# gkaissis/PriMIA

Hardware: AMD Instinct MI355X
Metric: images_per_sec (higher is better)
Workload: dtype bf16; 1 GPU; ResNet-18 federated-client training step (fwd+loss+bwd+SGD), batch 256/client, 3x224x224, 1 client per GPU; batch_per_client=256, clients=1, sync_every_n_batch=3, dp_sgd=False

## Files before the change

include/primia_hip.h:

```cpp
#ifndef PRIMIA_HIP_H
#define PRIMIA_HIP_H

#include <stdint.h>

#ifdef __cplusplus
extern "C" {
#endif

#define PRIMIA_OK 0
#define PRIMIA_ERR_ARG (-1)
#define PRIMIA_ERR_LAUNCH (-2)
#define PRIMIA_ERR_UNSUPPORTED (-3)
#define PRIMIA_ERR_WORKSPACE (-4)
#define PRIMIA_ERR_INTERNAL (-5)

#define PRIMIA_F32 0
#define PRIMIA_BF16 1

typedef void* primia_stream_t;

int primia_abi_version(void);

int primia_set_option(const char* name, int value);
int64_t primia_options_epoch(void);
// ... 21 lines not shown

int64_t primia_conv_wfwd_elems(const primia_conv_desc* d);
int64_t primia_conv_wdgrad_elems(const primia_conv_desc* d);

int primia_conv_weight_prepare(const primia_conv_desc* d, int c_real, const float* w_oihw,
                               void* w_fwd, void* w_dgrad, int dtype, primia_stream_t stream);

int primia_conv_weight_prepare_many(const primia_conv_desc* descs_host, const int* c_real_host,
                                    const float* const* w_oihw_host, void* const* w_fwd_host,
                                    void* const* w_dgrad_host, int n, int dtype, primia_stream_t stream);
int primia_conv_wgrad_finalize_many(const primia_conv_desc* descs_host, const int* c_real_host,
                                    const float* const* dw_acc_host, float* const* dw_oihw_host, int n,
                                    primia_stream_t stream);

int primia_conv_sgd_fusable(const primia_conv_desc* d, int c_real);
int primia_conv_sgd_step_many(const primia_conv_desc* descs_host, const int* c_real_host,
                              const float* const* dw_acc_host, float* const* dw_oihw_host,
                              float* const* w_oihw_host, void* const* w_fwd_host, void* const* w_dgrad_host,
                              int n, float lr, float weight_decay, int dtype, primia_stream_t stream);
int primia_conv_sgd_step_many_dev(const primia_conv_desc* descs_host, const int* c_real_host,
                                  const float* const* dw_acc_host, float* const* dw_oihw_host,
                                  float* const* w_oihw_host, void* const* w_fwd_host, void* const* w_dgrad_host,
                                  int n, const float* hyper, int dtype, primia_stream_t stream);

int primia_conv_fwd_pair_ok(const primia_conv_desc* d, const primia_conv_desc* d_ds, int dtype);
int primia_conv2d_fwd_stats_pair(const primia_conv_desc* d, const void* x, const void* w_fwd, void* y,
                                 float* stat_sums, const primia_conv_desc* d_ds, const void* w_fwd_ds, void* y_ds,
                                 float* stat_sums_ds, int dtype, primia_stream_t stream);

int primia_conv2d_fwd(const primia_conv_desc* d, const void* x, const void* w_fwd, void* y,
                      int dtype, primia_stream_t stream);
int primia_stem_pad_dims(int H, int W, int* Hp, int* Wp);
int primia_stem_conv_fwd(const void* x_padded, const void* w_fwd, void* y, int N, int H, int W, int dtype,
                         primia_stream_t stream);
int primia_stem_conv_stat_slots(int N, int H, int W);
int primia_stem_conv_fwd_stats(const void* x_padded, const void* w_fwd, void* y, float* stat_partials, int N, int H,
                               int W, int dtype, primia_stream_t stream);
int primia_stem_conv_stats(const void* x_padded, const void* w_fwd, float* stat_partials, int N, int H, int W, int dtype,
                           primia_stream_t stream);
int primia_stem_conv_pool_ok(int N, int H, int W, int dtype);
int primia_stem_conv_pool(const void* x_padded, const void* w_fwd, void* y, void* pooled, uint8_t* argmax,
                          const float* gamma, const float* beta, const float* save_mean, const float* save_invstd, int N,
                          int H, int W, int dtype, primia_stream_t stream);
int primia_stem_conv_pool_eval(const void* x_padded, const void* w_fwd, void* pooled, uint8_t* argmax, const float* gamma,
                               const float* beta, const float* running_mean, const float* running_var, float eps, int N,
                               int H, int W, int dtype, primia_stream_t stream);
// ... 288 lines not shown
                              float* ps_dbeta, int N, int HW, int C, void* workspace, int64_t workspace_bytes, int dtype,
                              primia_stream_t stream);

int primia_maxpool3x3s2_fwd(const void* x, void* y, uint8_t* argmax, int N, int H, int W, int C,
                            int dtype, primia_stream_t stream);
int primia_maxpool3x3s2_bwd(const void* dy, const uint8_t* argmax, void* dx, int N, int H, int W,
                            int C, int dtype, primia_stream_t stream);
int primia_avgpool3x3s2_fwd(const void* x, void* y, int N, int H, int W, int C, int dtype,
                            primia_stream_t stream);
int primia_avgpool3x3s2_bwd(const void* dy, void* dx, int N, int H, int W, int C, int dtype,
                            primia_stream_t stream);
int primia_global_avgpool_fwd(const void* x, float* feat, int N, int HW, int C, int dtype,
                              primia_stream_t stream);
int primia_global_avgpool_bwd(const float* dfeat, void* dx, int N, int HW, int C, int dtype,
                              primia_stream_t stream);

int primia_head_fwd(const void* x, const float* w, const float* b, float* feat, float* logits, int N, int HW, int C,
                    int out_f, int dtype, primia_stream_t stream);
int primia_head_bwd(const float* w, const float* dlogits, void* dx, int N, int HW, int C, int out_f, int dtype,
                    primia_stream_t stream);
int primia_head_bwd_bnsums(const float* w, const float* dlogits, void* dx, const void* bn_y, const uint8_t* relu_mask,
                           const float* bn_mean, const float* bn_invstd, float* sums, int N, int HW, int C, int out_f, int dtype,
                           primia_stream_t stream);
int primia_linear_fwd(const float* x, const float* w, const float* b, float* y, int N, int in_f,
                      int out_f, primia_stream_t stream);
int primia_linear_bwd(const float* x, const float* w, const float* dy, float* dx, float* dw,
                      float* db, int N, int in_f, int out_f, primia_stream_t stream);
int primia_xent_hard(const float* logits, const int64_t* target, const float* class_weight,
                     float* loss, float* dlogits, int N, int C, primia_stream_t stream);
int primia_xent_soft(const float* logits, const float* target, const float* class_weight,
                     float* loss, float* dlogits, int N, int C, primia_stream_t stream);

int primia_sgd_step(float* p, const float* g, int64_t n, float lr, float weight_decay,
                    primia_stream_t stream);
int primia_sgd_step_ranges(float* p, const float* g, const int64_t* begin_host, const int64_t* len_host, int n,
                           float lr, float weight_decay, primia_stream_t stream);
int primia_adam_step(float* p, const float* g, float* exp_avg, float* exp_avg_sq, int64_t n,
                     float lr, float beta1, float beta2, float eps, float weight_decay,
                     int64_t step, primia_stream_t stream);

int primia_sgd_step_dev(float* p, const float* g, int64_t n, const float* hyper, primia_stream_t stream);
int primia_sgd_step_ranges_dev(float* p, const float* g, const int64_t* begin_host, const int64_t* len_host, int n,
                               const float* hyper, primia_stream_t stream);
int primia_adam_step_dev(float* p, const float* g, float* exp_avg, float* exp_avg_sq, int64_t n,
                         const float* hyper, primia_stream_t stream);
int primia_opt_hyper_set(float* hyper, float lr, float weight_decay, float beta1, float beta2, float eps,
// ... 139 lines not shown
```

primia_amd/csrc/bn.hip:

```cpp
#include <stdlib.h>

#include "common.h"

namespace primia {

constexpr int kMaxPartialBlocks = 1024;


template <typename T, typename F, int UNROLL = 0>
__global__ __launch_bounds__(256) void colreduce2_kernel(F f, long M, int C, long rows_per_block,
                                                         float* __restrict__ partials) {
    constexpr int CH = Chunk<T>::N;
    const int tpr = C / CH;
    const int rpp = 256 / tpr;
    const int rg = threadIdx.x / tpr, cc = threadIdx.x % tpr;
    const long r0 = (long)blockIdx.x * rows_per_block;
    long r1 = r0 + rows_per_block;
    if (r1 > M) r1 = M;

    float s1[CH], s2[CH];
#pragma unroll
    for (int i = 0; i < CH; ++i) s1[i] = s2[i] = 0.f;
    if (rg < rpp) {
        F lf = f;
// ... 87 lines not shown

constexpr int kFinSlices = 64;
template <int NQ>
__device__ __forceinline__ void fin_gather(const float* __restrict__ partials, int nblk, int C, int c, int ks,
                                           double (&acc)[NQ]) {
    for (int k0 = ks; k0 < nblk; k0 += 8 * kFinSlices) {
        float v[8][NQ];
#pragma unroll
        for (int u = 0; u < 8; ++u) {
            const int k = k0 + u * kFinSlices;
#pragma unroll
            for (int q = 0; q < NQ; ++q) {
                const float t = partials[((long)(k < nblk ? k : nblk - 1) * NQ + q) * C + c];
                v[u][q] = k < nblk ? t : 0.f;
            }
        }
#pragma unroll
        for (int u = 0; u < 8; ++u)
#pragma unroll
            for (int q = 0; q < NQ; ++q) acc[q] += (double)v[u][q];
    }
}

__global__ __launch_bounds__(16 * kFinSlices) void bn_finalize_kernel(const float* __restrict__ partials, int nblk,
                                                          int C, long M, int mode, float eps,
                                                          float momentum, float* out1, float* out2,
                                                          float* running_mean, float* running_var,
                                                          const float* scale2 = nullptr) {
    __shared__ double sa[kFinSlices][17], sb[kFinSlices][17];
    const int cl = threadIdx.x & 15, ks = threadIdx.x >> 4;
    const int c = blockIdx.x * 16 + cl;
    float rm0 = 0.f, rv0 = 0.f, sc2v = 1.f;
    if (ks == 0 && c < C) {
        if (mode == 0 && running_mean) {
            rm0 = running_mean[c];
            rv0 = running_var[c];
        } else if (mode != 0 && scale2) {
            sc2v = scale2[c];
        }
    }
    double acc2[2] = {0.0, 0.0};
    if (c < C) fin_gather<2>(partials, nblk, C, c, ks, acc2);
    double a = acc2[0], b = acc2[1];
    sa[ks][cl] = a;
    sb[ks][cl] = b;
    __syncthreads();
    if (ks >= 4) return;
    for (int k = ks + 4; k < kFinSlices; k += 4) {
        a += sa[k][cl];
        b += sb[k][cl];
    }
    a += __shfl_down(a, 32);
    b += __shfl_down(b, 32);
    a += __shfl_down(a, 16);
    b += __shfl_down(b, 16);
    if (ks != 0 || c >= C) return;
    if (mode == 0) {
        const double mean = a / (double)M;
        double var = b / (double)M - mean * mean;
        if (var < 0.0) var = 0.0;
        out1[c] = (float)mean;
        out2[c] = (float)(1.0 / sqrt(var + (double)eps));
        if (running_mean) {
            const double unb = M > 1 ? var * (double)M / (double)(M - 1) : var;
            running_mean[c] = (float)((1.0 - momentum) * (double)rm0 + (double)momentum * mean);
            running_var[c] = (float)((1.0 - momentum) * (double)rv0 + (double)momentum * unb);
        }
    } else {
        out1[c] = (float)a;
        out2[c] = scale2 ? (float)(b * (double)sc2v) : (float)b;
    }
}

template <typename T>
__global__ __launch_bounds__(16 * kFinSlices) void bn_finalize_pool_kernel(
    const float* __restrict__ partials, int nblk, int C, float* __restrict__ dbeta, float* __restrict__ dgamma,
    const float* __restrict__ gamma, const float* __restrict__ beta, const float* __restrict__ mean,
    const float* __restrict__ invstd, const T* __restrict__ p, const T* __restrict__ dp, const uint8_t* __restrict__ argmax,
    const T* __restrict__ y, int N, int H, int W, int Ho, int Wo) {
    __shared__ double sa[kFinSlices][17], sb[kFinSlices][17];
    __shared__ double sfix[16 * kFinSlices / 64];
    const int cl = threadIdx.x & 15, ks = threadIdx.x >> 4;
    const int c = blockIdx.x * 16 + cl;
    double acc2[2] = {0.0, 0.0};
    if (c < C) fin_gather<2>(partials, nblk, C, c, ks, acc2);
    sa[ks][cl] = acc2[0];
    sb[ks][cl] = acc2[1];
    __syncthreads();
    if (ks == 0 && c < C) {
        double a = 0.0, b = 0.0;
        for (int k = 0; k < kFinSlices; ++k) {
            a += sa[k][cl];
            b += sb[k][cl];
        }
// ... 992 lines not shown
            (const T*)y, (const T*)dpooled, argmax, (T*)dy, gamma, beta, save_mean, save_invstd, dbeta, dgamma,
            (float)(1.0 / (double)M), N, H, W, C, Ho, Wo);
    } else {
        bn_relu_pool_bwd_apply_kernel<T><<<stream_blocks(nchunks) * 2, 256, 0, st>>>(
            (const T*)y, (const T*)dpooled, argmax, (T*)dy, gamma, beta, save_mean, save_invstd, dbeta, dgamma,
            (float)(1.0 / (double)M), N, H, W, C, Ho, Wo, 1.0f / (float)W, 1.0f / (float)H);
    }
    return launch_status();
}

}

using namespace primia;

template <typename T>
static int bn_fwd_train_pair_impl(const void* y2, const void* yd, void* z, uint8_t* relu_mask, const float* gamma2,
                                  const float* beta2, float* rm2, float* rv2, float* sm2, float* si2, const float* sums2,
                                  int slots2, const float* gammad, const float* betad, float* rmd, float* rvd, float* smd,
                                  float* sid, const float* sumsd, int slotsd, long M, int C, float eps, float momentum,
                                  float* ws, hipStream_t st) {
    int nblk;
    long rpb;
    reduce_geometry(M, C, nblk, rpb);
    const float* partd = sumsd;
    int nd = slotsd;
    if (!sumsd) {
        StatsFn<T> fd{(const T*)yd};
        colreduce2_kernel<T, StatsFn<T>><<<nblk, 256, 0, st>>>(fd, M, C, rpb, ws);
        partd = ws;
        nd = nblk;
    }
    bn_finalize_kernel<<<(C + 15) / 16, 16 * kFinSlices, 0, st>>>(partd, nd, C, M, 0, eps, momentum, smd, sid, rmd, rvd);
    const float* part = sums2;
    int n2 = slots2;
    if (!sums2) {
        StatsFn<T> f2{(const T*)y2};
        colreduce2_kernel<T, StatsFn<T>><<<nblk, 256, 0, st>>>(f2, M, C, rpb, ws);
        part = ws;
        n2 = nblk;
    }
    bn_finalize_kernel<<<(C + 15) / 16, 16 * kFinSlices, 0, st>>>(part, n2, C, M, 0, eps, momentum, sm2, si2, rm2, rv2);
    const long nchunks = M * C / Chunk<T>::N;
    bn_apply_pair_kernel<T><<<stream_blocks(nchunks), 256, 0, st>>>((const T*)y2, (const T*)yd, (T*)z, gamma2, beta2, sm2,
                                                                    si2, gammad, betad, smd, sid, nchunks, C, relu_mask);
    return launch_status();
}

extern "C" {

int64_t primia_bn_workspace_bytes(int64_t M, int C) {
    (void)M;
    return (int64_t)kMaxPartialBlocks * 2 * C * sizeof(float);
}

int primia_bn_fwd_train(const void* y, const void* residual, void* z, const float* gamma,
                        const float* beta, float* running_mean, float* running_var,
                        float* save_mean, float* save_invstd, int64_t M, int C, float eps,
                        float momentum, int relu, void* workspace, int64_t workspace_bytes,
                        int dtype, primia_stream_t stream) {
    PRIMIA_REQUIRE(y && z && gamma && beta && save_mean && save_invstd && workspace);
    PRIMIA_REQUIRE((running_mean == nullptr) == (running_var == nullptr));
    PRIMIA_REQUIRE(bn_shape_ok(M, C, dtype));
    if (workspace_bytes < primia_bn_workspace_bytes(M, C)) return PRIMIA_ERR_WORKSPACE;
    hipStream_t st = (hipStream_t)stream;
    if (dtype == PRIMIA_F32)
// ... 403 lines not shown
```

primia_amd/csrc/layout.hip:

```cpp
#include "common.h"
#include "conv_common.h"

namespace primia {

template <typename T>
__global__ __launch_bounds__(256) void nchw_to_nhwc_kernel(const float* __restrict__ src,
                                                           T* __restrict__ dst, int C, int HW,
                                                           int c_pad, long total) {
    long i = (long)blockIdx.x * blockDim.x + threadIdx.x;
    if (i >= total) return;
    long n = i / HW;
    long hw = i - n * HW;
    const float* s = src + n * (long)C * HW + hw;
    T* d = dst + i * c_pad;
    for (int c = 0; c < c_pad; ++c) Elem<T>::store(d + c, c < C ? s[(long)c * HW] : 0.f);
}

template <typename T>
__global__ __launch_bounds__(256) void nchw_to_nhwc_padded_kernel(const float* __restrict__ src, T* __restrict__ dst,
                                                                  int C, int H, int W, int c_pad, int pad_top,
                                                                  int pad_left, int Hp, int Wp, long total) {
    long i = (long)blockIdx.x * blockDim.x + threadIdx.x;
    if (i >= total) return;
    const int HW = H * W;
// ... 360 lines not shown
}

template <typename T>
__global__ __launch_bounds__(256) void conv_sgd_tiled_dev_kernel(SgdTileArgs a, const float* __restrict__ hyper) {
    __shared__ float lds[kTileK9 * (64 * 9 + 1)];
    const float lr = hyper[kHyperLr], wd = hyper[kHyperWd];
    int c = 0;
    while (c + 1 < a.n && (int)blockIdx.x >= a.tile_begin[c + 1]) ++c;
    const SgdTileEntry& en = a.e[c];
    const int tile = blockIdx.x - a.tile_begin[c];
    if (en.RS == 9)
        sgd_tile<T, 9, kTileK9, true>(en, tile, lds, lr, wd);
    else
        sgd_tile<T, 1, 32, true>(en, tile, lds, lr, wd);
}

constexpr int kMaxRanges = 32;
struct SgdRanges {
    long begin[kMaxRanges], len[kMaxRanges];
    int n;
    long total;
};
__device__ __forceinline__ void sgd_ranges_body(float* __restrict__ p, const float* __restrict__ g, const SgdRanges& r,
                                                float lr, float wd) {
    const long stride = (long)gridDim.x * 256;
    for (long i = (long)blockIdx.x * 256 + threadIdx.x; i < r.total; i += stride) {
        long j = i;
        int k = 0;
        while (k + 1 < r.n && j >= r.len[k]) j -= r.len[k++];
        const long o = r.begin[k] + j;
        p[o] = sgd_update(p[o], g[o], lr, wd);
    }
}
__global__ __launch_bounds__(256) void sgd_ranges_kernel(float* __restrict__ p, const float* __restrict__ g, SgdRanges r,
                                                         float lr, float wd) {
    sgd_ranges_body(p, g, r, lr, wd);
}
__global__ __launch_bounds__(256) void sgd_ranges_dev_kernel(float* __restrict__ p, const float* __restrict__ g,
                                                             SgdRanges r, const float* __restrict__ hyper) {
    const float lr = hyper[kHyperLr], wd = hyper[kHyperWd];
    sgd_ranges_body(p, g, r, lr, wd);
}

static inline bool tiled_ok(const ConvGeom& g, int c_real) {
    return !g.stem && c_real == g.C && g.C % 64 == 0 && g.K % 32 == 0 && (g.R * g.S == 9 || g.R * g.S == 1);
}

}

using namespace primia;

extern "C" {

int primia_abi_version(void) { return 1; }

int primia_nchw_to_nhwc(const float* src, void* dst, int N, int C, int H, int W, int c_pad,
                        int dtype, primia_stream_t stream) {
    PRIMIA_REQUIRE(src && dst && N > 0 && C > 0 && H > 0 && W > 0 && c_pad >= C);
    long total = (long)N * H * W;
    dim3 grid(ceil_div(total, 256)), block(256);
    hipStream_t st = (hipStream_t)stream;
    if (dtype == PRIMIA_F32)
        nchw_to_nhwc_kernel<float><<<grid, block, 0, st>>>(src, (float*)dst, C, H * W, c_pad, total);
    else if (dtype == PRIMIA_BF16)
        nchw_to_nhwc_kernel<bf16><<<grid, block, 0, st>>>(src, (bf16*)dst, C, H * W, c_pad, total);
    else
        return PRIMIA_ERR_ARG;
    return launch_status();
// ... 284 lines not shown
}

int primia_sgd_step_ranges(float* p, const float* g, const int64_t* begin_host, const int64_t* len_host, int n, float lr,
                           float weight_decay, primia_stream_t stream) {
    if (n == 0) return PRIMIA_OK;
    SgdRanges r;
    const int rc = sgd_ranges_args(p, g, begin_host, len_host, n, r);
    if (rc != PRIMIA_OK) return rc;
    sgd_ranges_kernel<<<sgd_ranges_blocks(r), 256, 0, (hipStream_t)stream>>>(p, g, r, lr, weight_decay);
    return launch_status();
}

int primia_sgd_step_ranges_dev(float* p, const float* g, const int64_t* begin_host, const int64_t* len_host, int n,
                               const float* hyper, primia_stream_t stream) {
    if (n == 0) return PRIMIA_OK;
    PRIMIA_REQUIRE(hyper);
    SgdRanges r;
    const int rc = sgd_ranges_args(p, g, begin_host, len_host, n, r);
    if (rc != PRIMIA_OK) return rc;
    sgd_ranges_dev_kernel<<<sgd_ranges_blocks(r), 256, 0, (hipStream_t)stream>>>(p, g, r, hyper);
    return launch_status();
}

}
```

primia_amd/csrc/pool_fc_loss.hip:

```cpp
#include "common.h"

namespace primia {

template <typename T, bool IS_MAX>
__global__ __launch_bounds__(256) void pool3x3s2_fwd_kernel(const T* __restrict__ x, T* __restrict__ y,
                                                            uint8_t* __restrict__ argmax, int N, int H,
                                                            int W, int C, int Ho, int Wo) {
    constexpr int CH = Chunk<T>::N;
    const int cpr = C / CH;
    const long total = (long)N * Ho * Wo * cpr;
    const long q = (long)blockIdx.x * 256 + threadIdx.x;
    if (q >= total) return;
    const int cc = (int)(q % cpr);
    long t = q / cpr;
    const int wo = (int)(t % Wo);
    t /= Wo;
    const int ho = (int)(t % Ho);
    const int n = (int)(t / Ho);
    float best[CH];
    int pos[CH];
#pragma unroll
    for (int i = 0; i < CH; ++i) {
        best[i] = IS_MAX ? -INFINITY : 0.f;
        pos[i] = -1;
// ... 116 lines not shown
__global__ __launch_bounds__(64) void linear_fwd_kernel(const float* __restrict__ x, const float* __restrict__ w,
                                                        const float* __restrict__ b, float* __restrict__ y,
                                                        int in_f, int out_f) {
    const int n = blockIdx.x, lane = threadIdx.x;
    for (int j = 0; j < out_f; ++j) {
        float s = 0.f;
        for (int i = lane; i < in_f; i += 64) s += x[(long)n * in_f + i] * w[(long)j * in_f + i];
        s = wave_sum(s);
        if (lane == 0) y[(long)n * out_f + j] = s + (b ? b[j] : 0.f);
    }
}
__global__ __launch_bounds__(256) void linear_bwd_dx_kernel(const float* __restrict__ w,
                                                            const float* __restrict__ dy,
                                                            float* __restrict__ dx, int N, int in_f,
                                                            int out_f) {
    const long i = (long)blockIdx.x * 256 + threadIdx.x;
    if (i >= (long)N * in_f) return;
    const int f = (int)(i % in_f);
    const long n = i / in_f;
    float s = 0.f;
    for (int j = 0; j < out_f; ++j) s += dy[n * out_f + j] * w[(long)j * in_f + f];
    dx[i] = s;
}
__global__ __launch_bounds__(1024) void linear_bwd_dw_kernel(const float* __restrict__ x,
                                                             const float* __restrict__ dy,
                                                             float* __restrict__ dw, float* __restrict__ db,
                                                             int N, int in_f, int out_f) {
    __shared__ float red[16][64];
    const int j = blockIdx.y, i = blockIdx.x * 64 + (threadIdx.x & 63), ng = threadIdx.x >> 6;
    float s = 0.f;
    if (i <= in_f)
        for (int n = ng; n < N; n += 16) s += dy[(long)n * out_f + j] * (i < in_f ? x[(long)n * in_f + i] : 1.f);
    red[ng][threadIdx.x & 63] = s;
    __syncthreads();
    if (ng == 0 && i <= in_f) {
        for (int g = 1; g < 16; ++g) s += red[g][threadIdx.x & 63];
        if (i < in_f)
            dw[(long)j * in_f + i] = s;
        else if (db)
            db[j] = s;
    }
}

template <typename T>
__global__ __launch_bounds__(256) void head_fwd_kernel(const T* __restrict__ x, const float* __restrict__ w,
                                                       const float* __restrict__ b, float* __restrict__ feat,
                                                       float* __restrict__ y, int HW, int C, int out_f) {
    constexpr int CH = Chunk<T>::N;
    extern __shared__ float sh[];
    const int tpr = C / CH, rpp = 256 / tpr;
    const int rg = threadIdx.x / tpr, cc = threadIdx.x % tpr;
    const int n = blockIdx.x;
    float s[CH];
#pragma unroll
    for (int i = 0; i < CH; ++i) s[i] = 0.f;
// ... 29 lines not shown
template <typename T>
__global__ __launch_bounds__(256) void head_bwd_kernel(const float* __restrict__ w, const float* __restrict__ dy,
                                                       T* __restrict__ dx, int HW, int C, int out_f) {
    constexpr int CH = Chunk<T>::N;
    extern __shared__ float sh[];
    const int n = blockIdx.x;
    for (int c = threadIdx.x; c < C; c += 256) {
        float a = 0.f;
        for (int j = 0; j < out_f; ++j) a += dy[(long)n * out_f + j] * w[(long)j * C + c];
        sh[c] = a / (float)HW;
    }
    __syncthreads();
    const int cpr = C / CH;
    for (int q = threadIdx.x; q < HW * cpr; q += 256) {
        const int c0 = (q % cpr) * CH;
        float v[CH];
#pragma unroll
        for (int i = 0; i < CH; ++i) v[i] = sh[c0 + i];
        *(u32x4*)(dx + (long)n * HW * C + (long)q * CH) = Chunk<T>::pack(v);
    }
}

template <typename T>
__global__ __launch_bounds__(256) void head_bwd_bnsums_kernel(const float* __restrict__ w, const float* __restrict__ dy,
                                                              T* __restrict__ dx, const T* __restrict__ bn_y,
                                                              const uint8_t* __restrict__ relu_mask,
                                                              const float* __restrict__ bn_mean,
                                                              const float* __restrict__ bn_invstd, float* __restrict__ sums,
                                                              int HW, int C, int out_f) {
    constexpr int CH = Chunk<T>::N;
    extern __shared__ float sh[];
    const int n = blockIdx.x;
    for (int c = threadIdx.x; c < C; c += 256) {
        float a = 0.f;
        for (int j = 0; j < out_f; ++j) a += dy[(long)n * out_f + j] * w[(long)j * C + c];
        sh[c] = a / (float)HW;
    }
    __syncthreads();
    const int cpr = C / CH;
    const int c0 = (threadIdx.x % cpr) * CH;
    float v[CH], vr[CH], mu[CH], cnt[CH], sx[CH];
#pragma unroll
    for (int i = 0; i < CH; ++i) {
        v[i] = sh[c0 + i];
        mu[i] = bn_mean[c0 + i];
        cnt[i] = sx[i] = 0.f;
    }
    const u32x4 packed = Chunk<T>::pack(v);
    Chunk<T>::unpack(packed, vr);
    for (int q = threadIdx.x; q < HW * cpr; q += 256) {
        const long off = (long)n * HW * C + (long)q * CH;
        *(u32x4*)(dx + off) = packed;
        float yv[CH];
        Chunk<T>::unpack(*(const u32x4*)(bn_y + off), yv);
        const unsigned m = relu_mask[off / CH];
#pragma unroll
        for (int i = 0; i < CH; ++i) {
            const bool on = (m >> i) & 1u;
            cnt[i] += on ? 1.f : 0.f;
            sx[i] += on ? yv[i] - mu[i] : 0.f;
        }
    }
    float* red = sh + C;
    const int grp = threadIdx.x / cpr;
#pragma unroll
    for (int i = 0; i < CH; ++i) {
        red[(grp * 2 + 0) * C + c0 + i] = vr[i] * cnt[i];
        red[(grp * 2 + 1) * C + c0 + i] = vr[i] * sx[i];
    }
    __syncthreads();
    const int ngrp = 256 / cpr;
    for (int c = threadIdx.x; c < 2 * C; c += 256) {
        const int qq = c / C, cc = c - qq * C;
        float a = 0.f;
        for (int g = 0; g < ngrp; ++g) a += red[(g * 2 + qq) * C + cc];
        if (qq) a *= bn_invstd[cc];
        sums[((long)n * 2 + qq) * C + cc] = a;
    }
}

__device__ __forceinline__ float block_sum_256(float v, float* sh) {
    v = wave_sum(v);
    if ((threadIdx.x & 63) == 0) sh[threadIdx.x >> 6] = v;
    __syncthreads();
    const float r = sh[0] + sh[1] + sh[2] + sh[3];
    __syncthreads();
    return r;
}

constexpr int kMaxClasses = 16;

template <bool SOFT>
__global__ __launch_bounds__(256) void xent_kernel(const float* __restrict__ logits, const void* target,
                                                   const float* __restrict__ cw, float* __restrict__ loss,
                                                   float* __restrict__ dlogits, int N, int C) {
    __shared__ float sh[4];
    float num = 0.f, den = 0.f;
    for (int n = threadIdx.x; n < N; n += 256) {
        const float* o = logits + (long)n * C;
        float mx = o[0];
// ... 168 lines not shown
        head_bwd_kernel<bf16><<<N, 256, lds, st>>>(w, dlogits, (bf16*)dx, HW, C, out_f);
    return launch_status();
}

int primia_head_bwd_bnsums(const float* w, const float* dlogits, void* dx, const void* bn_y, const uint8_t* relu_mask,
                           const float* bn_mean, const float* bn_invstd, float* sums, int N, int HW, int C, int out_f, int dtype,
                           primia_stream_t stream) {
    PRIMIA_REQUIRE(w && dlogits && dx && bn_y && relu_mask && bn_mean && bn_invstd && sums && N > 0 && HW > 0 && C > 0 && out_f > 0);
    PRIMIA_REQUIRE((dtype == PRIMIA_F32 || dtype == PRIMIA_BF16) && head_shape_ok(C, dtype));
    const int cpr = C / (dtype == PRIMIA_F32 ? 4 : 8);
    if (cpr > 256 || 256 % cpr) return PRIMIA_ERR_UNSUPPORTED;
    hipStream_t st = (hipStream_t)stream;
    const size_t lds = (size_t)(1 + 2 * (256 / cpr)) * C * sizeof(float);
    if (lds > 48 * 1024) return PRIMIA_ERR_UNSUPPORTED;
    if (dtype == PRIMIA_F32)
        head_bwd_bnsums_kernel<float><<<N, 256, lds, st>>>(w, dlogits, (float*)dx, (const float*)bn_y, relu_mask, bn_mean,
                                                           bn_invstd, sums, HW, C, out_f);
    else
        head_bwd_bnsums_kernel<bf16><<<N, 256, lds, st>>>(w, dlogits, (bf16*)dx, (const bf16*)bn_y, relu_mask, bn_mean,
                                                          bn_invstd, sums, HW, C, out_f);
    return launch_status();
}

int primia_linear_fwd(const float* x, const float* w, const float* b, float* y, int N, int in_f,
                      int out_f, primia_stream_t stream) {
    PRIMIA_REQUIRE(x && w && y && N > 0 && in_f > 0 && out_f > 0);
    linear_fwd_kernel<<<N, 64, 0, (hipStream_t)stream>>>(x, w, b, y, in_f, out_f);
    return launch_status();
}
int primia_linear_bwd(const float* x, const float* w, const float* dy, float* dx, float* dw,
                      float* db, int N, int in_f, int out_f, primia_stream_t stream) {
    PRIMIA_REQUIRE(x && w && dy && dw && N > 0 && in_f > 0 && out_f > 0);
    hipStream_t st = (hipStream_t)stream;
    if (dx) linear_bwd_dx_kernel<<<ceil_div((long)N * in_f, 256), 256, 0, st>>>(w, dy, dx, N, in_f, out_f);
    linear_bwd_dw_kernel<<<dim3((in_f + 1 + 63) / 64, out_f), 1024, 0, st>>>(x, dy, dw, db, N, in_f, out_f);
    return launch_status();
}

int primia_xent_hard(const float* logits, const int64_t* target, const float* class_weight,
                     float* loss, float* dlogits, int N, int C, primia_stream_t stream) {
    PRIMIA_REQUIRE(logits && target && loss && N > 0 && C > 0);
    xent_kernel<false><<<1, 256, 0, (hipStream_t)stream>>>(logits, target, class_weight, loss, dlogits, N, C);
    return launch_status();
}
int primia_xent_soft(const float* logits, const float* target, const float* class_weight,
                     float* loss, float* dlogits, int N, int C, primia_stream_t stream) {
// ... 7 lines not shown
```

primia_amd/engine.py:

```python
import os
from collections import OrderedDict

import torch

from . import _lib
from ._lib import ConvDesc, call, query
from .resnet_spec import NetSpec, bn_name, buffer_entries, init_state_dict, param_entries, resnet18_spec, state_dict_keys

BN_EPS = 1e-5
BN_MOMENTUM = 0.1


class _Conv:
    def __init__(self, spec, desc, c_real):
        self.spec, self.desc, self.c_real = spec, desc, c_real


class ResNet18Engine:
    def __init__(self, batch_size, num_classes=3, in_channels=3, input_size=224, pooling="max",
                 dtype=torch.bfloat16, device="cuda:0", norm="batch", groups=32, options=None, share=None):
        self._root = self if share is None else share._root
        self._options = dict(options or {})
        for k, v in self._options.items():
            if not hasattr(type(self), k):
# ... 785 lines not shown
            smp, sip = self.save[pb2]
            self._timed("dgrad", c1, lambda: call(
                "primia_conv2d_dgrad_pair_bnsums", c1.desc, dy1, c1.w_dgrad, cd.desc, dyd, cd.w_dgrad, dx_in,
                t[prev.prefix + ".y2"], self.relu_masks[pb2], smp, sip, sums, self.dt), extra_macs=self._macs(cd))
            self._dout_sums[prev.prefix] = (sums, pslots)
        else:
            self._timed("dgrad", c1, lambda: call("primia_conv2d_dgrad_pair", c1.desc, dy1, c1.w_dgrad, cd.desc, dyd,
                                                  cd.w_dgrad, dx_in, self.dt), extra_macs=self._macs(cd))

    def backward(self):
        N, t = self.N, self.t
        nc = self.spec.num_classes
        if query("primia_options_epoch") != self._options_epoch:
            raise _lib.PrimiaError("library options changed (primia_set_option) after this engine sized its buffers")
        self._grads_pending = False
        self._wg_seen = {}
        self._dout_sums = {}
        if self.wgrad_ws is not None and self.dp is None:
            stem_overwrites = self._acc_zero_only_stem and self._stem_bwd_fused_wanted()
            if not stem_overwrites:
                self.dw_acc[:self._acc_zero_n].zero_()
        else:
            self.dw_acc.zero_()
        call("primia_linear_bwd", self.feat, self.views["fc.weight"], self.dlogits, None,
             self._gviews["fc.weight"], self._gviews["fc.bias"], N, 512, nc)
        last = self.spec.blocks[-1].prefix
        hw = self.final_hw
        blocks = self.spec.blocks
        lb2 = bn_name(blocks[-1].conv2.name)
        if (self.norm == "batch" and self.dp is None and blocks[-1].down is None and lb2 in self.relu_masks
                and self._head_bnsums_ok()):
            sums = self._bwd_sums("head", N, 512)
            sml, sil = self.save[lb2]
            call("primia_head_bwd_bnsums", self.views["fc.weight"], self.dlogits, t[last + ".dout"], t[last + ".y2"],
                 self.relu_masks[lb2], sml, sil, sums, N, hw * hw, 512, nc, self.dt)
            self._dout_sums[last] = (sums, N)
        else:
            call("primia_head_bwd", self.views["fc.weight"], self.dlogits, t[last + ".dout"], N, hw * hw, 512, nc, self.dt)
        for i in range(len(blocks) - 1, -1, -1):
            blk, prev = blocks[i], (blocks[i - 1] if i > 0 else None)
            x_in = t[prev.prefix + ".out"] if prev is not None else t["pool.out"]
            dx_in = t[prev.prefix + ".dout"] if prev is not None else t["pool.dout"]
            if self.taps is not None:
                self.taps[blk.prefix + ".dout_in"] = t[blk.prefix + ".dout"].clone()
            if blk.down is None:
                self._backward_identity(blk, prev, x_in, dx_in)
            else:
                self._backward_transition(blk, prev, x_in, dx_in)
        hw = self.stem_hw
        stem_bwd_fused = self._stem_bwd_fused_wanted()
        self.stem_bwd_fused_active = stem_bwd_fused
        pool_sums, self._pool_sums = getattr(self, "_pool_sums", None), None
        if stem_bwd_fused:
            sm, si = self.save["bn1"]
            c = self.convs["conv1"]
            S = self.spec.input_size
            if pool_sums is not None:
                call("primia_bn_relu_maxpool_bwd_from_sums", t["stem.y"], t["pool.out"], t["pool.dout"], self.pool_argmax,
                     self.views["bn1.weight"], self.views["bn1.bias"], sm, si, self._gviews["bn1.weight"],
                     self._gviews["bn1.bias"], pool_sums[0], pool_sums[1], N, hw, hw, 64, self.dt)
# ... 89 lines not shown
    def _sgd_tail_plan(self):
        if getattr(self, "_sgd_plan", None) is None:
            import ctypes

            cs = list(self.convs.values())
            fus = [c for c in cs if query("primia_conv_sgd_fusable", c.desc, c.c_real) == 1 and c.w_dgrad is not None
                   and all(tt.data_ptr() % 16 == 0 for tt in (c.acc, c.w_fwd, c.w_dgrad, self.views[c.spec.name + ".weight"],
                                                              self._gviews[c.spec.name + ".weight"]))]
            rest = [c for c in cs if c not in fus]
            vp = lambda t: ctypes.c_void_p(t.data_ptr()) if t is not None else ctypes.c_void_p(0)

            def pack(lst):
                n = len(lst)
                if n == 0:
                    return None
                return dict(
                    n=n, descs=(ConvDesc * n)(*[c.desc for c in lst]), creal=(ctypes.c_int * n)(*[c.c_real for c in lst]),
                    w=(ctypes.c_void_p * n)(*[vp(self.views[c.spec.name + ".weight"]) for c in lst]),
                    wf=(ctypes.c_void_p * n)(*[vp(c.w_fwd) for c in lst]),
                    wd=(ctypes.c_void_p * n)(*[vp(c.w_dgrad) for c in lst]),
                    acc=(ctypes.c_void_p * n)(*[vp(c.acc) for c in lst]),
                    gw=(ctypes.c_void_p * n)(*[vp(self._gviews[c.spec.name + ".weight"]) for c in lst]))

            fused_keys = {c.spec.name + ".weight" for c in fus}
            ranges, off = [], 0
            for k, shp in self.p_entries:
                n = int(torch.Size(shp).numel())
                if k not in fused_keys:
                    if ranges and ranges[-1][0] + ranges[-1][1] == off:
                        ranges[-1][1] += n
                    else:
                        ranges.append([off, n])
                off += n
            if not fus or len(ranges) > 32:
                self._sgd_plan = False
            else:
                nr = len(ranges)
                self._sgd_plan = (pack(fus), pack(rest), (ctypes.c_int64 * nr)(*[r[0] for r in ranges]),
                                  (ctypes.c_int64 * nr)(*[r[1] for r in ranges]), nr)
        return self._sgd_plan or None

    @property
    def grads(self):
        self.materialize_grads()
        return self._grads

    def materialize_grads(self):
        if self._grads_pending:
            m = self._many_args()
            call("primia_conv_wgrad_finalize_many", m["descs"], m["creal"], m["acc"], m["gw"], m["n"])
            self._grads_pending = False

    def dp_loss_backward(self, target, max_grad_norm=1.0, noise_multiplier=1.3, noise=None, generator=None):
        if self.norm not in ("group", "frozen"):
            raise _lib.PrimiaError("DP-SGD needs per-sample independent norm layers: ResNet18Engine(norm='group') or "
                                   "norm='frozen' (BatchNorm with fixed statistics)")
        N, nc, dev = self.N, self.spec.num_classes, self.device
        call("primia_xent_hard", self.logits, target, None, self.loss, self.dlogits, N, nc)
        call("primia_scale", self.dlogits, self.dlogits.numel(), float(N))
        self.dp = {"wgrads": []}
        try:
            self.backward()
# ... 143 lines not shown
                    else:
                        n = query("primia_conv_wgrad_persample_slab_bytes", self.convs[c.name].desc, self.dt)
                    if n > 0:
                        self._dp_keep[c.name] = torch.empty(n // 4, dtype=torch.float32, device=self.device)
        return self._dp_keep

    def zero_grad(self):
        self._grads_pending = False
        self.grads.zero_()

    def note_replayed_steps(self, n):
        if self.norm != "frozen":
            for b in self.num_batches_tracked:
                self.num_batches_tracked[b] += int(n)
        if self.opt_state is not None:
            self.opt_steps += int(n)

    def reset_optimizer(self):
        self.opt_state = None
        self.opt_steps = 0

    def sgd_step(self, lr, weight_decay=0.0, hyper=None):
        if self._grads_pending:
            fus, rest, rb, rl, nr = self._sgd_tail_plan()
            self._grads_pending = False
            if hyper is None:
                call("primia_conv_sgd_step_many", fus["descs"], fus["creal"], fus["acc"], fus["gw"], fus["w"], fus["wf"],
                     fus["wd"], fus["n"], float(lr), float(weight_decay), self.dt)
            else:
                call("primia_conv_sgd_step_many_dev", fus["descs"], fus["creal"], fus["acc"], fus["gw"], fus["w"],
                     fus["wf"], fus["wd"], fus["n"], hyper, self.dt)
            if rest is not None:
                call("primia_conv_wgrad_finalize_many", rest["descs"], rest["creal"], rest["acc"], rest["gw"], rest["n"])
            if hyper is None:
                call("primia_sgd_step_ranges", self.flat, self._grads, rb, rl, nr, float(lr), float(weight_decay))
            else:
                call("primia_sgd_step_ranges_dev", self.flat, self._grads, rb, rl, nr, hyper)
            if rest is not None:
                call("primia_conv_weight_prepare_many", rest["descs"], rest["creal"], rest["w"], rest["wf"], rest["wd"],
                     rest["n"], self.dt)
            return
        if hyper is None:
            call("primia_sgd_step", self.flat, self.grads, self.P, float(lr), float(weight_decay))
        else:
            call("primia_sgd_step_dev", self.flat, self.grads, self.P, hyper)
        self.refresh_weights()

    def adam_step(self, lr, betas=(0.9, 0.999), eps=1e-8, weight_decay=0.0, hyper=None):
# ... 19 lines not shown
```

Before: 56180 images/s.

## Fuse optimizer tail, head backward with fc grads, and paired BN finalize into single launches

Merges the conv-weight SGD tiles, the stem weight update and repack, and the flat-range SGD for the remaining parameters into one kernel launch. It also folds the fc weight and bias gradient into the head backward BN-sums kernel, and finalizes both BN statistics of a residual pair in a single launch. The aim is to cut kernel launch count and small-kernel tail overhead in each training step. In exchange the kernels get more complex, with block-index dispatch and heterogeneous blocks that may load-balance unevenly.

```diff
diff --git a/include/primia_hip.h b/include/primia_hip.h
--- a/include/primia_hip.h
+++ b/include/primia_hip.h
@@ -67,6 +67,17 @@
                                   const float* const* dw_acc_host, float* const* dw_oihw_host,
                                   float* const* w_oihw_host, void* const* w_fwd_host, void* const* w_dgrad_host,
                                   int n, const float* hyper, int dtype, primia_stream_t stream);
+
+int primia_conv_sgd_tail_fusable(const primia_conv_desc* d, int c_real);
+int primia_sgd_tail(const primia_conv_desc* descs_host, const int* c_real_host, const float* const* dw_acc_host,
+                    float* const* dw_oihw_host, float* const* w_oihw_host, void* const* w_fwd_host,
+                    void* const* w_dgrad_host, int n, float* p, const float* g, const int64_t* begin_host,
+                    const int64_t* len_host, int n_ranges, float lr, float weight_decay, int dtype,
+                    primia_stream_t stream);
+int primia_sgd_tail_dev(const primia_conv_desc* descs_host, const int* c_real_host, const float* const* dw_acc_host,
+                        float* const* dw_oihw_host, float* const* w_oihw_host, void* const* w_fwd_host,
+                        void* const* w_dgrad_host, int n, float* p, const float* g, const int64_t* begin_host,
+                        const int64_t* len_host, int n_ranges, const float* hyper, int dtype, primia_stream_t stream);
 
 int primia_conv_fwd_pair_ok(const primia_conv_desc* d, const primia_conv_desc* d_ds, int dtype);
 int primia_conv2d_fwd_stats_pair(const primia_conv_desc* d, const void* x, const void* w_fwd, void* y,
@@ -401,6 +412,9 @@
 int primia_head_bwd_bnsums(const float* w, const float* dlogits, void* dx, const void* bn_y, const uint8_t* relu_mask,
                            const float* bn_mean, const float* bn_invstd, float* sums, int N, int HW, int C, int out_f, int dtype,
                            primia_stream_t stream);
+int primia_head_bwd_bnsums_dw(const float* w, const float* dlogits, void* dx, const void* bn_y, const uint8_t* relu_mask,
+                              const float* bn_mean, const float* bn_invstd, float* sums, const float* feat, float* dw,
+                              float* db, int N, int HW, int C, int out_f, int dtype, primia_stream_t stream);
 int primia_linear_fwd(const float* x, const float* w, const float* b, float* y, int N, int in_f,
                       int out_f, primia_stream_t stream);
 int primia_linear_bwd(const float* x, const float* w, const float* dy, float* dx, float* dw,
diff --git a/primia_amd/csrc/bn.hip b/primia_amd/csrc/bn.hip
--- a/primia_amd/csrc/bn.hip
+++ b/primia_amd/csrc/bn.hip
@@ -133,14 +133,12 @@
     }
 }
 
-__global__ __launch_bounds__(16 * kFinSlices) void bn_finalize_kernel(const float* __restrict__ partials, int nblk,
-                                                          int C, long M, int mode, float eps,
-                                                          float momentum, float* out1, float* out2,
-                                                          float* running_mean, float* running_var,
-                                                          const float* scale2 = nullptr) {
+__device__ __forceinline__ void bn_finalize_body(const float* __restrict__ partials, int nblk, int C, long M, int mode,
+                                                 float eps, float momentum, float* out1, float* out2, float* running_mean,
+                                                 float* running_var, const float* scale2, int cblk) {
     __shared__ double sa[kFinSlices][17], sb[kFinSlices][17];
     const int cl = threadIdx.x & 15, ks = threadIdx.x >> 4;
-    const int c = blockIdx.x * 16 + cl;
+    const int c = cblk * 16 + cl;
     float rm0 = 0.f, rv0 = 0.f, sc2v = 1.f;
     if (ks == 0 && c < C) {
         if (mode == 0 && running_mean) {
@@ -181,6 +179,28 @@
         out1[c] = (float)a;
         out2[c] = scale2 ? (float)(b * (double)sc2v) : (float)b;
     }
+}
+
+__global__ __launch_bounds__(16 * kFinSlices) void bn_finalize_kernel(const float* __restrict__ partials, int nblk,
+                                                          int C, long M, int mode, float eps,
+                                                          float momentum, float* out1, float* out2,
+                                                          float* running_mean, float* running_var,
+                                                          const float* scale2 = nullptr) {
+    bn_finalize_body(partials, nblk, C, M, mode, eps, momentum, out1, out2, running_mean, running_var, scale2, blockIdx.x);
+}
+
+struct BnFinTable {
+    const float* partials;
+    int nblk;
+    float *mean, *invstd, *running_mean, *running_var;
+};
+__global__ __launch_bounds__(16 * kFinSlices) void bn_finalize_pair_kernel(BnFinTable t0, BnFinTable t1, int C, long M,
+                                                                           float eps, float momentum) {
+    const int nb = gridDim.x >> 1;
+    const bool second = (int)blockIdx.x >= nb;
+    const BnFinTable& t = second ? t1 : t0;
+    bn_finalize_body(t.partials, t.nblk, C, M, 0, eps, momentum, t.mean, t.invstd, t.running_mean, t.running_var, nullptr,
+                     second ? blockIdx.x - nb : blockIdx.x);
 }
 
 template <typename T>
@@ -1219,6 +1239,14 @@
     int nblk;
     long rpb;
     reduce_geometry(M, C, nblk, rpb);
+    const long nchunks = M * C / Chunk<T>::N;
+    if (sums2 && sumsd) {
+        const BnFinTable t0{sumsd, slotsd, smd, sid, rmd, rvd}, t1{sums2, slots2, sm2, si2, rm2, rv2};
+        bn_finalize_pair_kernel<<<2 * ((C + 15) / 16), 16 * kFinSlices, 0, st>>>(t0, t1, C, M, eps, momentum);
+        bn_apply_pair_kernel<T><<<stream_blocks(nchunks), 256, 0, st>>>((const T*)y2, (const T*)yd, (T*)z, gamma2, beta2, sm2,
+                                                                        si2, gammad, betad, smd, sid, nchunks, C, relu_mask);
+        return launch_status();
+    }
     const float* partd = sumsd;
     int nd = slotsd;
     if (!sumsd) {
@@ -1237,7 +1265,6 @@
         n2 = nblk;
     }
     bn_finalize_kernel<<<(C + 15) / 16, 16 * kFinSlices, 0, st>>>(part, n2, C, M, 0, eps, momentum, sm2, si2, rm2, rv2);
-    const long nchunks = M * C / Chunk<T>::N;
     bn_apply_pair_kernel<T><<<stream_blocks(nchunks), 256, 0, st>>>((const T*)y2, (const T*)yd, (T*)z, gamma2, beta2, sm2,
                                                                     si2, gammad, betad, smd, sid, nchunks, C, relu_mask);
     return launch_status();
diff --git a/primia_amd/csrc/layout.hip b/primia_amd/csrc/layout.hip
--- a/primia_amd/csrc/layout.hip
+++ b/primia_amd/csrc/layout.hip
@@ -406,9 +406,9 @@
     long total;
 };
 __device__ __forceinline__ void sgd_ranges_body(float* __restrict__ p, const float* __restrict__ g, const SgdRanges& r,
-                                                float lr, float wd) {
-    const long stride = (long)gridDim.x * 256;
-    for (long i = (long)blockIdx.x * 256 + threadIdx.x; i < r.total; i += stride) {
+                                                float lr, float wd, int blk, int nblk) {
+    const long stride = (long)nblk * 256;
+    for (long i = (long)blk * 256 + threadIdx.x; i < r.total; i += stride) {
         long j = i;
         int k = 0;
         while (k + 1 < r.n && j >= r.len[k]) j -= r.len[k++];
@@ -418,16 +418,69 @@
 }
 __global__ __launch_bounds__(256) void sgd_ranges_kernel(float* __restrict__ p, const float* __restrict__ g, SgdRanges r,
                                                          float lr, float wd) {
-    sgd_ranges_body(p, g, r, lr, wd);
+    sgd_ranges_body(p, g, r, lr, wd, blockIdx.x, gridDim.x);
 }
 __global__ __launch_bounds__(256) void sgd_ranges_dev_kernel(float* __restrict__ p, const float* __restrict__ g,
                                                              SgdRanges r, const float* __restrict__ hyper) {
     const float lr = hyper[kHyperLr], wd = hyper[kHyperWd];
-    sgd_ranges_body(p, g, r, lr, wd);
+    sgd_ranges_body(p, g, r, lr, wd, blockIdx.x, gridDim.x);
+}
+
+struct SgdStemEntry {
+    int K, c_real;
+    const float* acc;
+    float* grad;
+    float* w;
+    void* wf;
+};
+template <typename T>
+__device__ __forceinline__ void sgd_stem_block(const SgdStemEntry& en, int k, float* lds, float lr, float wd) {
+    const int n = en.c_real * 49, t = threadIdx.x;
+    if (t < n) {
+        const int c = t / 49, rs = t - c * 49, r = rs / 7, s_ = rs - r * 7;
+        const long o = (long)k * n + t;
+        const float g = en.acc[(long)k * 256 + r * 32 + s_ * 4 + c];
+        en.grad[o] = g;
+        const float wn = sgd_update(en.w[o], g, lr, wd);
+        en.w[o] = wn;
+        lds[t] = wn;
+    }
+    __syncthreads();
+    const int r = t >> 5, s_ = (t & 31) >> 2, c = t & 3;
+    float v = 0.f;
+    if (r < 7 && s_ < 7 && c < en.c_real) v = lds[(c * 7 + r) * 7 + s_];
+    Elem<T>::store((T*)en.wf + (long)k * 256 + t, v);
+}
+
+template <typename T, bool kDev>
+__global__ __launch_bounds__(256) void conv_sgd_tail_kernel(SgdTileArgs a, SgdStemEntry stem, float* __restrict__ p,
+                                                            const float* __restrict__ g, SgdRanges r,
+                                                            const float* __restrict__ hyper) {
+    __shared__ float lds[kTileK9 * (64 * 9 + 1)];
+    const float lr = kDev ? hyper[kHyperLr] : a.lr, wd = kDev ? hyper[kHyperWd] : a.wd;
+    const int tiles = a.tile_begin[a.n], b = blockIdx.x;
+    if (b < tiles) {
+        int c = 0;
+        while (c + 1 < a.n && b >= a.tile_begin[c + 1]) ++c;
+        const SgdTileEntry& en = a.e[c];
+        const int tile = b - a.tile_begin[c];
+        if (en.RS == 9)
+            sgd_tile<T, 9, kTileK9, kDev>(en, tile, lds, lr, wd);
+        else
+            sgd_tile<T, 1, 32, kDev>(en, tile, lds, lr, wd);
+    } else if (b < tiles + stem.K) {
+        sgd_stem_block<T>(stem, b - tiles, lds, lr, wd);
+    } else {
+        sgd_ranges_body(p, g, r, lr, wd, b - tiles - stem.K, (int)gridDim.x - tiles - stem.K);
+    }
 }
 
 static inline bool tiled_ok(const ConvGeom& g, int c_real) {
     return !g.stem && c_real == g.C && g.C % 64 == 0 && g.K % 32 == 0 && (g.R * g.S == 9 || g.R * g.S == 1);
+}
+
+static inline bool stem_tail_ok(const ConvGeom& g, int c_real) {
+    return g.stem && g.klen == 256 && c_real >= 1 && c_real <= 4;
 }
 
 }
@@ -758,4 +811,85 @@
     return launch_status();
 }
 
-}
+static int sgd_tail_launch(const primia_conv_desc* descs, const int* c_real, const float* const* dw_acc,
+                           float* const* dw_oihw, float* const* w_oihw, void* const* w_fwd, void* const* w_dgrad, int n,
+                           float* p, const float* g, const int64_t* begin_host, const int64_t* len_host, int n_ranges,
+                           float lr, float weight_decay, const float* hyper, int dtype, hipStream_t st) {
+    PRIMIA_REQUIRE(descs && c_real && dw_acc && dw_oihw && w_oihw && w_fwd && w_dgrad && n > 0 && n <= kMaxConvs + 1);
+    PRIMIA_REQUIRE(dtype == PRIMIA_F32 || dtype == PRIMIA_BF16);
+    primia_conv_desc tdesc[kMaxConvs];
+    int tc[kMaxConvs];
+    const float* tacc[kMaxConvs];
+    float *tgw[kMaxConvs], *tw[kMaxConvs];
+    void *twf[kMaxConvs], *twd[kMaxConvs];
+    int nt = 0;
+    SgdStemEntry stem{0, 0, nullptr, nullptr, nullptr, nullptr};
+    for (int i = 0; i < n; ++i) {
+        ConvGeom cg;
+        PRIMIA_REQUIRE(cg.init(descs[i]));
+        if (stem_tail_ok(cg, c_real[i])) {
+            PRIMIA_REQUIRE(dw_acc[i] && dw_oihw[i] && w_oihw[i] && w_fwd[i] && !w_dgrad[i]);
+            if (stem.K) return PRIMIA_ERR_UNSUPPORTED;
+            stem = SgdStemEntry{cg.K, c_real[i], dw_acc[i], dw_oihw[i], w_oihw[i], w_fwd[i]};
+        } else {
+            if (nt == kMaxConvs) return PRIMIA_ERR_ARG;
+            tdesc[nt] = descs[i]; tc[nt] = c_real[i]; tacc[nt] = dw_acc[i]; tgw[nt] = dw_oihw[i]; tw[nt] = w_oihw[i];
+            twf[nt] = w_fwd[i]; twd[nt] = w_dgrad[i];
+            ++nt;
+        }
+    }
+    SgdTileArgs ta;
+    int tiles = 0;
+    ta.n = 0;
+    ta.lr = lr;
+    ta.wd = weight_decay;
+    if (nt) {
+        const int rc = conv_sgd_args(tdesc, tc, tacc, tgw, tw, twf, twd, nt, lr, weight_decay, dtype, ta, tiles);
+        if (rc != PRIMIA_OK) return rc;
+    }
+    ta.tile_begin[ta.n] = tiles;
+    SgdRanges r;
+    r.n = 0;
+    r.total = 0;
+    int rblocks = 0;
+    if (n_ranges) {
+        const int rc = sgd_ranges_args(p, g, begin_host, len_host, n_ranges, r);
+        if (rc != PRIMIA_OK) return rc;
+        rblocks = sgd_ranges_blocks(r);
+    }
+    const int blocks = tiles + stem.K + rblocks;
+    if (dtype == PRIMIA_F32) {
+        if (hyper) conv_sgd_tail_kernel<float, true><<<blocks, 256, 0, st>>>(ta, stem, p, g, r, hyper);
+        else conv_sgd_tail_kernel<float, false><<<blocks, 256, 0, st>>>(ta, stem, p, g, r, nullptr);
+    } else {
+        if (hyper) conv_sgd_tail_kernel<bf16, true><<<blocks, 256, 0, st>>>(ta, stem, p, g, r, hyper);
+        else conv_sgd_tail_kernel<bf16, false><<<blocks, 256, 0, st>>>(ta, stem, p, g, r, nullptr);
+    }
+    return launch_status();
+}
+
+int primia_conv_sgd_tail_fusable(const primia_conv_desc* d, int c_real) {
+    if (!d) return PRIMIA_ERR_ARG;
+    ConvGeom g;
+    if (!g.init(*d)) return PRIMIA_ERR_ARG;
+    return (tiled_ok(g, c_real) || stem_tail_ok(g, c_real)) ? 1 : 0;
+}
+
+int primia_sgd_tail(const primia_conv_desc* descs, const int* c_real, const float* const* dw_acc, float* const* dw_oihw,
+                    float* const* w_oihw, void* const* w_fwd, void* const* w_dgrad, int n, float* p, const float* g,
+                    const int64_t* begin_host, const int64_t* len_host, int n_ranges, float lr, float weight_decay,
+                    int dtype, primia_stream_t stream) {
+    return sgd_tail_launch(descs, c_real, dw_acc, dw_oihw, w_oihw, w_fwd, w_dgrad, n, p, g, begin_host, len_host, n_ranges,
+                           lr, weight_decay, nullptr, dtype, (hipStream_t)stream);
+}
+
+int primia_sgd_tail_dev(const primia_conv_desc* descs, const int* c_real, const float* const* dw_acc,
+                        float* const* dw_oihw, float* const* w_oihw, void* const* w_fwd, void* const* w_dgrad, int n,
+                        float* p, const float* g, const int64_t* begin_host, const int64_t* len_host, int n_ranges,
+                        const float* hyper, int dtype, primia_stream_t stream) {
+    PRIMIA_REQUIRE(hyper);
+    return sgd_tail_launch(descs, c_real, dw_acc, dw_oihw, w_oihw, w_fwd, w_dgrad, n, p, g, begin_host, len_host, n_ranges,
+                           0.f, 0.f, hyper, dtype, (hipStream_t)stream);
+}
+
+}
diff --git a/primia_amd/csrc/pool_fc_loss.hip b/primia_amd/csrc/pool_fc_loss.hip
--- a/primia_amd/csrc/pool_fc_loss.hip
+++ b/primia_amd/csrc/pool_fc_loss.hip
@@ -162,15 +162,20 @@
     for (int j = 0; j < out_f; ++j) s += dy[n * out_f + j] * w[(long)j * in_f + f];
     dx[i] = s;
 }
+__device__ __forceinline__ float linear_dw_group(const float* __restrict__ x, const float* __restrict__ dy, int N, int in_f,
+                                                 int out_f, int j, int i, int ng) {
+    float s = 0.f;
+    if (i <= in_f)
+        for (int n = ng; n < N; n += 16) s += dy[(long)n * out_f + j] * (i < in_f ? x[(long)n * in_f + i] : 1.f);
+    return s;
+}
 __global__ __launch_bounds__(1024) void linear_bwd_dw_kernel(const float* __restrict__ x,
                                                              const float* __restrict__ dy,
                                                              float* __restrict__ dw, float* __restrict__ db,
                                                              int N, int in_f, int out_f) {
     __shared__ float red[16][64];
     const int j = blockIdx.y, i = blockIdx.x * 64 + (threadIdx.x & 63), ng = threadIdx.x >> 6;
-    float s = 0.f;
-    if (i <= in_f)
-        for (int n = ng; n < N; n += 16) s += dy[(long)n * out_f + j] * (i < in_f ? x[(long)n * in_f + i] : 1.f);
+    float s = linear_dw_group(x, dy, N, in_f, out_f, j, i, ng);
     red[ng][threadIdx.x & 63] = s;
     __syncthreads();
     if (ng == 0 && i <= in_f) {
@@ -246,14 +251,13 @@
 }
 
 template <typename T>
-__global__ __launch_bounds__(256) void head_bwd_bnsums_kernel(const float* __restrict__ w, const float* __restrict__ dy,
-                                                              T* __restrict__ dx, const T* __restrict__ bn_y,
-                                                              const uint8_t* __restrict__ relu_mask,
-                                                              const float* __restrict__ bn_mean,
-                                                              const float* __restrict__ bn_invstd, float* __restrict__ sums,
-                                                              int HW, int C, int out_f) {
+__device__ __forceinline__ void head_bwd_bnsums_body(const float* __restrict__ w, const float* __restrict__ dy,
+                                                     T* __restrict__ dx, const T* __restrict__ bn_y,
+                                                     const uint8_t* __restrict__ relu_mask,
+                                                     const float* __restrict__ bn_mean,
+                                                     const float* __restrict__ bn_invstd, float* __restrict__ sums,
+                                                     int HW, int C, int out_f, float* sh) {
     constexpr int CH = Chunk<T>::N;
-    extern __shared__ float sh[];
     const int n = blockIdx.x;
     for (int c = threadIdx.x; c < C; c += 256) {
         float a = 0.f;
@@ -300,6 +304,67 @@
         for (int g = 0; g < ngrp; ++g) a += red[(g * 2 + qq) * C + cc];
         if (qq) a *= bn_invstd[cc];
         sums[((long)n * 2 + qq) * C + cc] = a;
+    }
+}
+template <typename T>
+__global__ __launch_bounds__(256) void head_bwd_bnsums_kernel(const float* __restrict__ w, const float* __restrict__ dy,
+                                                              T* __restrict__ dx, const T* __restrict__ bn_y,
+                                                              const uint8_t* __restrict__ relu_mask,
+                                                              const float* __restrict__ bn_mean,
+                                                              const float* __restrict__ bn_invstd, float* __restrict__ sums,
+                                                              int HW, int C, int out_f) {
+    extern __shared__ float sh[];
+    head_bwd_bnsums_body<T>(w, dy, dx, bn_y, relu_mask, bn_mean, bn_invstd, sums, HW, C, out_f, sh);
+}
+
+template <typename T>
+__global__ __launch_bounds__(256) void head_bwd_bnsums_dw_kernel(const float* __restrict__ w, const float* __restrict__ dy,
+                                                                 T* __restrict__ dx, const T* __restrict__ bn_y,
+                                                                 const uint8_t* __restrict__ relu_mask,
+                                                                 const float* __restrict__ bn_mean,
+                                                                 const float* __restrict__ bn_invstd,
+                                                                 float* __restrict__ sums, const float* __restrict__ feat,
+                                                                 float* __restrict__ dw, float* __restrict__ db, int N,
+                                                                 int HW, int C, int out_f) {
+    extern __shared__ float sh[];
+    if ((int)blockIdx.x < N) {
+        head_bwd_bnsums_body<T>(w, dy, dx, bn_y, relu_mask, bn_mean, bn_invstd, sums, HW, C, out_f, sh);
+        return;
+    }
+    const int b = blockIdx.x - N, ncb = (C + 1 + 63) / 64;
+    const int j = b / ncb, lane = threadIdx.x & 63, wave = threadIdx.x >> 6;
+    const int i = (b - j * ncb) * 64 + lane;
+    float sg[4] = {0.f, 0.f, 0.f, 0.f};
+    if (i <= C) {
+        const int ic = i < C ? i : C - 1;
+        for (int n0 = 0; n0 < N; n0 += 64) {
+            float a[4][4], x[4][4];
+#pragma unroll
+            for (int u = 0; u < 4; ++u)
+#pragma unroll
+                for (int q = 0; q < 4; ++q) {
+                    const int n = n0 + 16 * u + wave + 4 * q, nc = n < N ? n : N - 1;
+                    a[u][q] = dy[(long)nc * out_f + j];
+                    const float f = feat[(long)nc * C + ic];
+                    x[u][q] = i < C ? f : 1.f;
+                }
+#pragma unroll
+            for (int u = 0; u < 4; ++u)
+#pragma unroll
+                for (int q = 0; q < 4; ++q)
+                    if (n0 + 16 * u + wave + 4 * q < N) sg[q] += a[u][q] * x[u][q];
+        }
+    }
+#pragma unroll
+    for (int q = 0; q < 4; ++q) sh[(wave + 4 * q) * 64 + lane] = sg[q];
+    __syncthreads();
+    if (wave == 0 && i <= C) {
+        float s = sg[0];
+        for (int g = 1; g < 16; ++g) s += sh[g * 64 + lane];
+        if (i < C)
+            dw[(long)j * C + i] = s;
+        else if (db)
+            db[j] = s;
     }
 }
 
@@ -514,6 +579,28 @@
     return launch_status();
 }
 
+int primia_head_bwd_bnsums_dw(const float* w, const float* dlogits, void* dx, const void* bn_y, const uint8_t* relu_mask,
+                              const float* bn_mean, const float* bn_invstd, float* sums, const float* feat, float* dw,
+                              float* db, int N, int HW, int C, int out_f, int dtype, primia_stream_t stream) {
+    PRIMIA_REQUIRE(w && dlogits && dx && bn_y && relu_mask && bn_mean && bn_invstd && sums && feat && dw && N > 0 && HW > 0 &&
+                   C > 0 && out_f > 0);
+    PRIMIA_REQUIRE((dtype == PRIMIA_F32 || dtype == PRIMIA_BF16) && head_shape_ok(C, dtype));
+    const int cpr = C / (dtype == PRIMIA_F32 ? 4 : 8);
+    if (cpr > 256 || 256 % cpr) return PRIMIA_ERR_UNSUPPORTED;
+    hipStream_t st = (hipStream_t)stream;
+    size_t lds = (size_t)(1 + 2 * (256 / cpr)) * C * sizeof(float);
+    if (lds > 48 * 1024) return PRIMIA_ERR_UNSUPPORTED;
+    if (lds < 16 * 64 * sizeof(float)) lds = 16 * 64 * sizeof(float);
+    const int blocks = N + (C + 1 + 63) / 64 * out_f;
+    if (dtype == PRIMIA_F32)
+        head_bwd_bnsums_dw_kernel<float><<<blocks, 256, lds, st>>>(w, dlogits, (float*)dx, (const float*)bn_y, relu_mask,
+                                                                   bn_mean, bn_invstd, sums, feat, dw, db, N, HW, C, out_f);
+    else
+        head_bwd_bnsums_dw_kernel<bf16><<<blocks, 256, lds, st>>>(w, dlogits, (bf16*)dx, (const bf16*)bn_y, relu_mask,
+                                                                  bn_mean, bn_invstd, sums, feat, dw, db, N, HW, C, out_f);
+    return launch_status();
+}
+
 int primia_linear_fwd(const float* x, const float* w, const float* b, float* y, int N, int in_f,
                       int out_f, primia_stream_t stream) {
     PRIMIA_REQUIRE(x && w && y && N > 0 && in_f > 0 && out_f > 0);
diff --git a/primia_amd/engine.py b/primia_amd/engine.py
--- a/primia_amd/engine.py
+++ b/primia_amd/engine.py
@@ -831,8 +831,6 @@
                 self.dw_acc[:self._acc_zero_n].zero_()
         else:
             self.dw_acc.zero_()
-        call("primia_linear_bwd", self.feat, self.views["fc.weight"], self.dlogits, None,
-             self._gviews["fc.weight"], self._gviews["fc.bias"], N, 512, nc)
         last = self.spec.blocks[-1].prefix
         hw = self.final_hw
         blocks = self.spec.blocks
@@ -841,10 +839,13 @@
                 and self._head_bnsums_ok()):
             sums = self._bwd_sums("head", N, 512)
             sml, sil = self.save[lb2]
-            call("primia_head_bwd_bnsums", self.views["fc.weight"], self.dlogits, t[last + ".dout"], t[last + ".y2"],
-                 self.relu_masks[lb2], sml, sil, sums, N, hw * hw, 512, nc, self.dt)
+            call("primia_head_bwd_bnsums_dw", self.views["fc.weight"], self.dlogits, t[last + ".dout"], t[last + ".y2"],
+                 self.relu_masks[lb2], sml, sil, sums, self.feat, self._gviews["fc.weight"], self._gviews["fc.bias"],
+                 N, hw * hw, 512, nc, self.dt)
             self._dout_sums[last] = (sums, N)
         else:
+            call("primia_linear_bwd", self.feat, self.views["fc.weight"], self.dlogits, None,
+                 self._gviews["fc.weight"], self._gviews["fc.bias"], N, 512, nc)
             call("primia_head_bwd", self.views["fc.weight"], self.dlogits, t[last + ".dout"], N, hw * hw, 512, nc, self.dt)
         for i in range(len(blocks) - 1, -1, -1):
             blk, prev = blocks[i], (blocks[i - 1] if i > 0 else None)
@@ -980,22 +981,34 @@
                     acc=(ctypes.c_void_p * n)(*[vp(c.acc) for c in lst]),
                     gw=(ctypes.c_void_p * n)(*[vp(self._gviews[c.spec.name + ".weight"]) for c in lst]))
 
-            fused_keys = {c.spec.name + ".weight" for c in fus}
-            ranges, off = [], 0
-            for k, shp in self.p_entries:
-                n = int(torch.Size(shp).numel())
-                if k not in fused_keys:
-                    if ranges and ranges[-1][0] + ranges[-1][1] == off:
-                        ranges[-1][1] += n
-                    else:
-                        ranges.append([off, n])
-                off += n
+            def ranges_outside(lst):
+                keys = {c.spec.name + ".weight" for c in lst}
+                ranges, off = [], 0
+                for k, shp in self.p_entries:
+                    n = int(torch.Size(shp).numel())
+                    if k not in keys:
+                        if ranges and ranges[-1][0] + ranges[-1][1] == off:
+                            ranges[-1][1] += n
+                        else:
+                            ranges.append([off, n])
+                    off += n
+                return ranges
+
+            i64 = lambda v: (ctypes.c_int64 * len(v))(*v)
+            ranges = ranges_outside(fus)
+            single = None
+            if fus and len(rest) <= 1 and len(cs) <= 25 and all(
+                    query("primia_conv_sgd_tail_fusable", c.desc, c.c_real) == 1 and c.w_dgrad is None
+                    and query("primia_conv_sgd_fusable", c.desc, c.c_real) != 1 for c in rest):
+                r1 = ranges_outside(cs)
+                if 0 < len(r1) <= 32:
+                    single = (pack(fus + rest), i64([r[0] for r in r1]), i64([r[1] for r in r1]), len(r1))
             if not fus or len(ranges) > 32:
                 self._sgd_plan = False
             else:
                 nr = len(ranges)
-                self._sgd_plan = (pack(fus), pack(rest), (ctypes.c_int64 * nr)(*[r[0] for r in ranges]),
-                                  (ctypes.c_int64 * nr)(*[r[1] for r in ranges]), nr)
+                self._sgd_plan = (pack(fus), pack(rest), i64([r[0] for r in ranges]), i64([r[1] for r in ranges]), nr,
+                                  single)
         return self._sgd_plan or None
 
     @property
@@ -1185,8 +1198,17 @@
 
     def sgd_step(self, lr, weight_decay=0.0, hyper=None):
         if self._grads_pending:
-            fus, rest, rb, rl, nr = self._sgd_tail_plan()
+            fus, rest, rb, rl, nr, single = self._sgd_tail_plan()
             self._grads_pending = False
+            if single is not None:
+                m, sb, sl, sn = single
+                if hyper is None:
+                    call("primia_sgd_tail", m["descs"], m["creal"], m["acc"], m["gw"], m["w"], m["wf"], m["wd"], m["n"],
+                         self.flat, self._grads, sb, sl, sn, float(lr), float(weight_decay), self.dt)
+                else:
+                    call("primia_sgd_tail_dev", m["descs"], m["creal"], m["acc"], m["gw"], m["w"], m["wf"], m["wd"],
+                         m["n"], self.flat, self._grads, sb, sl, sn, hyper, self.dt)
+                return
             if hyper is None:
                 call("primia_conv_sgd_step_many", fus["descs"], fus["creal"], fus["acc"], fus["gw"], fus["w"], fus["wf"],
                      fus["wd"], fus["n"], float(lr), float(weight_decay), self.dt)
```

Measured after the change: 56520 images/s (median of 6 runs). About the same (+0.6%).
